# felicityin/zkvm-brainfuck

Hardware: AMD Instinct MI355X
Metric: core-proof wall-time (ms) + NTT HBM GB/s, fibonacci trace 2^22 rows (lower is better)
Workload: dtype u32 (KoalaBear mod-p); 1 GPU; fibo_x4 stdin[255]: 3,767,729 cycles, Cpu trace 2^22 rows, full core proof (84 FRI queries, 16 PoW bits); cycles=3767729, parallelism=replicas x1

## Files before the change

zkvm-brainfuck_amd/csrc/merkle.hip:

```cpp
#include <algorithm>

#include "merkle.h"
#include "poseidon2.h"


namespace bfz {

using namespace kb;

constexpr int MAXSEG = 16;
struct ColList {
  const uint32_t* base[MAXSEG];
  size_t stride[MAXSEG];
  int start[MAXSEG + 1];
  int nseg;
  int n;
  __device__ __forceinline__ const uint32_t* col(int c) const {
    int s = 0;
    while (s + 1 < nseg && c >= start[s + 1]) s++;
    return base[s] + (size_t)(c - start[s]) * stride[s];
  }
};

__device__ __forceinline__ void sponge_cols(uint32_t st[16], const ColList& cl, size_t row) {
  for (int c0 = 0; c0 < cl.n; c0 += 8) {
#pragma unroll
    for (int k = 0; k < 8; k++)
      if (c0 + k < cl.n) st[k] = cl.col(c0 + k)[row];
    poseidon2_permute(st);
  }
}

__global__ __launch_bounds__(256) void k_hash_leaves(ColList cl, size_t r0, size_t count,
                                                     uint32_t* __restrict__ out) {
  const size_t i = (size_t)blockIdx.x * blockDim.x + threadIdx.x;
  if (i >= count) return;
  const size_t r = r0 + i;
  uint32_t st[16];
#pragma unroll
  for (int i = 0; i < 16; i++) st[i] = 0;
  sponge_cols(st, cl, r);
  uint4* o = reinterpret_cast<uint4*>(out + 8 * r);
  o[0] = make_uint4(st[0], st[1], st[2], st[3]);
  o[1] = make_uint4(st[4], st[5], st[6], st[7]);
}

__device__ __forceinline__ void merkle_node(uint32_t st[16], const ColList& cl, int c0, int c1,
                                            size_t j) {
  const int nchunks = (c1 - c0 + 7) >> 3;
  const int nsteps = nchunks ? nchunks + 2 : 1;
  uint32_t d[8];
  for (int step = 0; step < nsteps; step++) {
    if (step == 1) {
#pragma unroll
      for (int i = 0; i < 8; i++) d[i] = st[i];
#pragma unroll
      for (int i = 0; i < 16; i++) st[i] = 0;
    }
    if (step >= 1 && step <= nchunks) {
      const int cb = c0 + 8 * (step - 1);
#pragma unroll
      for (int k = 0; k < 8; k++)
        if (cb + k < c1) st[k] = cl.col(cb + k)[j];
    }
    if (nchunks && step == nchunks + 1) {
#pragma unroll
      for (int i = 0; i < 8; i++) {
        st[8 + i] = st[i];
        st[i] = d[i];
      }
    }
    poseidon2_permute(st);
  }
}

__device__ __forceinline__ void load16(uint32_t st[16], const uint32_t* p) {
  const uint4* in = reinterpret_cast<const uint4*>(p);
  const uint4 a = in[0], b = in[1], c = in[2], d = in[3];
  st[0] = a.x; st[1] = a.y; st[2] = a.z; st[3] = a.w;
  st[4] = b.x; st[5] = b.y; st[6] = b.z; st[7] = b.w;
  st[8] = c.x; st[9] = c.y; st[10] = c.z; st[11] = c.w;
  st[12] = d.x; st[13] = d.y; st[14] = d.z; st[15] = d.w;
}

__device__ __forceinline__ void store8(uint32_t* p, const uint32_t st[16]) {
  uint4* o = reinterpret_cast<uint4*>(p);
  o[0] = make_uint4(st[0], st[1], st[2], st[3]);
  o[1] = make_uint4(st[4], st[5], st[6], st[7]);
}

__global__ __launch_bounds__(256) void k_compress(const uint32_t* __restrict__ prev, size_t j0,
                                                  size_t count, uint32_t* __restrict__ out,
                                                  ColList inj) {
  const size_t i = (size_t)blockIdx.x * blockDim.x + threadIdx.x;
  if (i >= count) return;
  const size_t j = j0 + i;
  uint32_t st[16];
  load16(st, prev + 16 * j);
  merkle_node(st, inj, 0, inj.n, j);
  store8(out + 8 * j, st);
}

__device__ __forceinline__ uint32_t merkle_node_lane(uint32_t v, const ColList& cl, int c0, int c1,
                                                     size_t j, int lane, const LaneConsts& kc) {
  v = poseidon2_permute_lane(v, lane, kc);
  const int nchunks = (c1 - c0 + 7) >> 3;
  if (nchunks) {
    const uint32_t d = v;
    uint32_t h = 0;
    for (int k = 0; k < nchunks; k++) {
      const int col = c0 + 8 * k + lane;
      if (lane < 8 && col < c1) h = cl.col(col)[j];
      h = poseidon2_permute_lane(h, lane, kc);
    }
    const uint32_t hs = dpp<DPP_ROR8>(h);
    v = poseidon2_permute_lane(lane < 8 ? d : hs, lane, kc);
  }
  return v;
}

constexpr int TOP_NODES = 64;
constexpr int TOP_LAYERS = 7;
constexpr size_t LANE_LAYER_MAX = (size_t)1 << 14;
constexpr int MAXTOP = TOP_LAYERS;
struct TopLayers {
  uint32_t* out[MAXTOP];
  int c0[MAXTOP], c1[MAXTOP];
  int n;
};

__global__ __launch_bounds__(1024) void k_compress_top(const uint32_t* __restrict__ prev,
                                                       size_t nlen, ColList inj, TopLayers tl,
                                                       RootChallenge rc, size_t base) {
  __shared__ uint32_t buf[2][TOP_NODES * 8];
  const size_t per = nlen < (size_t)TOP_NODES ? nlen : (size_t)TOP_NODES;
  const size_t g0 = base + (size_t)blockIdx.x * per;
  const int lane = threadIdx.x & 15;
  const LaneConsts kc = lane_consts(lane);
  for (int l = 0; l < tl.n; l++) {
    const size_t m = per >> l, g = g0 >> l;
    const uint32_t* src = buf[(l - 1) & 1];
    uint32_t* dst = buf[l & 1];
    for (size_t j = threadIdx.x >> 4; j < m; j += blockDim.x >> 4) {
      const uint32_t x = l == 0 ? ld_global(prev, 16 * (g + j) + lane) : src[16 * j + lane];
      const uint32_t v = merkle_node_lane(x, inj, tl.c0[l], tl.c1[l], g + j, lane, kc);
      if (lane < 8) {
        tl.out[l][8 * (g + j) + lane] = v;
        dst[8 * j + lane] = v;
      }
    }
    __syncthreads();
  }
  if (rc.state && threadIdx.x < 64) {
    const uint32_t* root = buf[(tl.n - 1) & 1];
    uint32_t v = lane < 8 ? root[lane] : ld_global(rc.state, lane);
    v = poseidon2_permute_lane(v, lane, kc);
    if (threadIdx.x < 16) {
      rc.state[lane] = v;
      if (lane >= 4 && lane < 8) rc.beta->c[7 - lane] = v;
    }
  }
}

__global__ __launch_bounds__(256) void k_compress_lanes(const uint32_t* __restrict__ prev,
                                                        size_t j0, size_t count,
                                                        uint32_t* __restrict__ out, ColList inj) {
  const size_t i = ((size_t)blockIdx.x * blockDim.x + threadIdx.x) >> 4;
  const int lane = threadIdx.x & 15;
  if (i >= count) return;
  const size_t j = j0 + i;
  const uint32_t v = merkle_node_lane(prev[16 * j + lane], inj, 0, inj.n, j, lane, lane_consts(lane));
  if (lane < 8) out[8 * j + lane] = v;
}

__global__ __launch_bounds__(256) void k_hash_rows8_lanes(const uint32_t* __restrict__ rows,
                                                          size_t r0, size_t count,
                                                          uint32_t* __restrict__ out) {
  const size_t i = r0 + (((size_t)blockIdx.x * blockDim.x + threadIdx.x) >> 4);
  const int lane = threadIdx.x & 15;
  if (i >= r0 + count) return;
  const uint32_t v = poseidon2_permute_lane(lane < 8 ? rows[8 * i + lane] : 0u, lane);
  if (lane < 8) out[8 * i + lane] = v;
}

__global__ __launch_bounds__(256) void k_permute_lanes(uint32_t* __restrict__ s, size_t n) {
  const size_t i = ((size_t)blockIdx.x * blockDim.x + threadIdx.x) >> 4;
  const int lane = threadIdx.x & 15;
  if (i >= n) return;
  s[16 * i + lane] = poseidon2_permute_lane(s[16 * i + lane], lane);
}

__global__ __launch_bounds__(256) void k_permute_batch(uint32_t* __restrict__ s, size_t n) {
  const size_t i = (size_t)blockIdx.x * blockDim.x + threadIdx.x;
  if (i >= n) return;
  uint32_t st[16];
#pragma unroll
  for (int k = 0; k < 16; k++) st[k] = s[16 * i + k];
  poseidon2_permute(st);
#pragma unroll
  for (int k = 0; k < 16; k++) s[16 * i + k] = st[k];
}

__global__ __launch_bounds__(256) void k_hash_rows8(const uint32_t* __restrict__ rows, size_t r0,
                                                    size_t count, uint32_t* __restrict__ out) {
  const size_t i = r0 + (size_t)blockIdx.x * blockDim.x + threadIdx.x;
  if (i >= r0 + count) return;
  uint32_t st[16];
  const uint4* in = reinterpret_cast<const uint4*>(rows + 8 * i);
  uint4 a = in[0], b = in[1];
  st[0] = a.x; st[1] = a.y; st[2] = a.z; st[3] = a.w;
  st[4] = b.x; st[5] = b.y; st[6] = b.z; st[7] = b.w;
#pragma unroll
  for (int k = 8; k < 16; k++) st[k] = 0;
  poseidon2_permute(st);
  uint4* o = reinterpret_cast<uint4*>(out + 8 * i);
  o[0] = make_uint4(st[0], st[1], st[2], st[3]);
  o[1] = make_uint4(st[4], st[5], st[6], st[7]);
}

static ColList make_cols(const std::vector<const MatRef*>& ms) {
  ColList cl{};
  cl.n = 0;
  cl.nseg = 0;
  for (const MatRef* m : ms) {
    if (cl.nseg >= MAXSEG) throw std::runtime_error("merkle: too many matrices at one height");
    cl.base[cl.nseg] = m->base;
    cl.stride[cl.nseg] = m->stride ? m->stride : m->height;
    cl.start[cl.nseg] = cl.n;
    cl.nseg++;
    cl.n += m->width;
  }
  cl.start[cl.nseg] = cl.n;
  return cl;
}

static void launch_layer(MerkleTree& t, int L, size_t j0, size_t count,
                         const std::vector<const MatRef*>& grp, hipStream_t st) {
  const uint32_t* prev = t.layers[L - 1].p;
  if (count <= LANE_LAYER_MAX)
    hipLaunchKernelGGL(k_compress_lanes, dim3(ceil_div(16 * count, 256)), dim3(256), 0, st, prev,
                       j0, count, t.layers[L].p, make_cols(grp));
  else {
    const ColList cl = make_cols(grp);
    KernelProbe& probe = p2_probe();
    hipEvent_t ev0 = probe.on ? probe.begin(st) : nullptr;
    hipLaunchKernelGGL(k_compress, dim3(ceil_div(count, 256)), dim3(256), 0, st, prev, j0, count,
                       t.layers[L].p, cl);
    if (probe.on)
      probe.end(ev0, st, (double)count * (cl.n ? 2 + (cl.n + 7) / 8 : 1), cl.n ? "k_compress+inject" : "k_compress");
  }
  KCHECK();
}

static void build_layers(MerkleTree& t, int L0, size_t len, const std::vector<const MatRef*>& sorted,
                         size_t next, hipStream_t st, bool fetch_root = true,
                         RootChallenge rc = {}) {
  const int nl = (int)t.layers.size() - 1;
  int L = L0;
  for (; L <= nl && (len >> 1) > LANE_LAYER_MAX; L++) {
    const size_t nlen = len >> 1;
    std::vector<const MatRef*> grp;
    while (next < sorted.size() && sorted[next]->height == nlen) grp.push_back(sorted[next++]);
    t.layers[L].reset(8 * nlen);
    launch_layer(t, L, 0, nlen, grp, st);
    len = nlen;
  }
  while (L <= nl) {
    const size_t first = len >> 1;
    const int sub = first > (size_t)TOP_NODES ? TOP_LAYERS : log2i(first) + 1;
    TopLayers tl{};
    tl.n = std::min(sub, nl - L + 1);
    std::vector<const MatRef*> all;
    size_t nlen = first;
    for (int l = 0; l < tl.n; l++, nlen >>= 1) {
      tl.c0[l] = 0;
      for (const MatRef* m : all) tl.c0[l] += m->width;
      while (next < sorted.size() && sorted[next]->height == nlen) all.push_back(sorted[next++]);
      tl.c1[l] = 0;
      for (const MatRef* m : all) tl.c1[l] += m->width;
      t.layers[L + l].reset(8 * nlen);
      tl.out[l] = t.layers[L + l].p;
    }
    const unsigned blocks = first > (size_t)TOP_NODES ? (unsigned)(first / TOP_NODES) : 1u;
    const bool root_launch = L + tl.n > nl;
    hipLaunchKernelGGL(k_compress_top, dim3(blocks), dim3(16 * TOP_NODES), 0, st,
                       (const uint32_t*)t.layers[L - 1].p, first, make_cols(all), tl,
                       root_launch ? rc : RootChallenge{}, (size_t)0);
    KCHECK();
    L += tl.n;
    len = first >> (tl.n - 1);
  }
  if (next != sorted.size()) throw std::runtime_error("merkle: non power-of-two heights");
  if (!fetch_root) return;
  fetch(t.root, t.layers[nl].p, 32, st);
}

ShardCtx*& shard_ctx() {
  static ShardCtx* c = nullptr;
  return c;
}

static bool shard_tree(size_t h0) {
  const ShardCtx* c = shard_ctx();
  return c && c->world > 1 && h0 >= (size_t)c->world * SHARD_MIN_LEAVES;
}

template <class Leaves>
static void build_sharded(MerkleTree& t, size_t h0, const std::vector<const MatRef*>& sorted,
                          size_t next, Leaves leaves, hipStream_t st, bool fetch_root,
                          RootChallenge rc = {}) {
  const ShardCtx& c = *shard_ctx();
  const size_t G = (size_t)c.world, k = (size_t)c.rank;
  const int nl = log2i(h0), lg = log2i(G);
  t.sharded_below = nl - lg;
  t.shard_log = lg;
  leaves(k * (h0 / G), h0 / G);
  size_t len = h0;
  int L = 1;
  for (; L <= nl - lg && (len >> 1) / G > LANE_LAYER_MAX; L++) {
    const size_t nlen = len >> 1;
    std::vector<const MatRef*> grp;
    while (next < sorted.size() && sorted[next]->height == nlen) grp.push_back(sorted[next++]);
    t.layers[L].reset(8 * nlen);
    launch_layer(t, L, k * (nlen / G), nlen / G, grp, st);
    len = nlen;
  }
  while (L <= nl - lg) {
    const size_t first = (len >> 1) / G;
    const int sub = first > (size_t)TOP_NODES ? TOP_LAYERS : log2i(first) + 1;
    TopLayers tl{};
    tl.n = std::min(sub, nl - lg - L + 1);
    std::vector<const MatRef*> all;
    size_t nlen = len >> 1;
    for (int l = 0; l < tl.n; l++, nlen >>= 1) {
      tl.c0[l] = 0;
      for (const MatRef* m : all) tl.c0[l] += m->width;
      while (next < sorted.size() && sorted[next]->height == nlen) all.push_back(sorted[next++]);
      tl.c1[l] = 0;
      for (const MatRef* m : all) tl.c1[l] += m->width;
      t.layers[L + l].reset(8 * nlen);
      tl.out[l] = t.layers[L + l].p;
    }
    const unsigned blocks = first > (size_t)TOP_NODES ? (unsigned)(first / TOP_NODES) : 1u;
    hipLaunchKernelGGL(k_compress_top, dim3(blocks), dim3(16 * TOP_NODES), 0, st,
                       (const uint32_t*)t.layers[L - 1].p, first, make_cols(all), tl,
                       RootChallenge{}, k * first);
    KCHECK();
    L += tl.n;
    len >>= tl.n;
  }
  DBuf<uint32_t>& lay = t.layers[nl - lg];
  DBuf<uint32_t> all(8 * G);
  coll_sync(st);
  c.allgather(lay.p + 8 * k, 32, all.p);
  HIP_CHECK(hipMemcpyAsync(lay.p, all.p, 32 * G, hipMemcpyDeviceToDevice, st));
  build_layers(t, nl - lg + 1, G, sorted, next, st, fetch_root, rc);
}

void merkle_build(const std::vector<MatRef>& mats, MerkleTree& t, hipStream_t st, bool fetch_root) {
  if (mats.empty()) throw std::runtime_error("merkle: no matrices");
  t.mats = mats;
  std::vector<const MatRef*> sorted;
  for (const MatRef& m : mats) sorted.push_back(&m);
  std::stable_sort(sorted.begin(), sorted.end(),
                   [](const MatRef* a, const MatRef* b) { return a->height > b->height; });
  const size_t h0 = sorted[0]->height;
  t.layers.clear();
  t.layers.resize(log2i(h0) + 1);
  t.sharded_below = 0;
  size_t next = 0;
  std::vector<const MatRef*> grp;
  while (next < sorted.size() && sorted[next]->height == h0) grp.push_back(sorted[next++]);
  t.layers[0].reset(8 * h0);
  const ColList cl = make_cols(grp);
  auto leaves = [&](size_t r0, size_t count) {
    KernelProbe& probe = p2_probe();
    hipEvent_t ev0 = probe.on ? probe.begin(st) : nullptr;
    hipLaunchKernelGGL(k_hash_leaves, dim3(ceil_div(count, 256)), dim3(256), 0, st, cl, r0,
                       count, t.layers[0].p);
    KCHECK();
    if (probe.on) probe.end(ev0, st, (double)count * ((cl.n + 7) / 8), "k_hash_leaves");
  };
  if (shard_tree(h0)) {
    build_sharded(t, h0, sorted, next, leaves, st, fetch_root);
    return;
  }
  leaves(0, h0);
  build_layers(t, 1, h0, sorted, next, st, fetch_root);
}

static void hash_rows8_range(const uint32_t* rows, size_t r0, size_t count, uint32_t* digests,
                             hipStream_t st) {
  if (count <= LANE_LAYER_MAX)
    hipLaunchKernelGGL(k_hash_rows8_lanes, dim3(ceil_div(16 * count, 256)), dim3(256), 0, st, rows,
                       r0, count, digests);
  else {
    KernelProbe& probe = p2_probe();
    hipEvent_t ev0 = probe.on ? probe.begin(st) : nullptr;
    hipLaunchKernelGGL(k_hash_rows8, dim3(ceil_div(count, 256)), dim3(256), 0, st, rows, r0, count,
                       digests);
    if (probe.on) probe.end(ev0, st, (double)count, "k_hash_rows8");
  }
  KCHECK();
}

void merkle_from_rows8(MerkleTree& t, const uint32_t* rows, size_t h, hipStream_t st,
                       bool fetch_root, RootChallenge rc, bool allow_shard,
                       const std::function<void(size_t, size_t, uint32_t*)>& fused) {
  t.mats = {MatRef{rows, h, 8}};
  t.layers.clear();
  t.layers.resize(log2i(h) + 1);
  t.layers[0].reset(8 * h);
  t.sharded_below = 0;
  auto leaves = [&](size_t r0, size_t count) {
    if (fused) fused(r0, count, t.layers[0].p);
    else hash_rows8_range(rows, r0, count, t.layers[0].p, st);
  };
  if (h < 2) throw std::runtime_error("merkle: rows8 tree needs two leaves");
  if (allow_shard && shard_tree(h)) {
    build_sharded(t, h, {}, 0, leaves, st, fetch_root, rc);
    return;
  }
  leaves(0, h);
  build_layers(t, 1, h, {}, 0, st, fetch_root, rc);
}

void poseidon2_batch(uint32_t* states, size_t n, hipStream_t st) {
  hipLaunchKernelGGL(k_permute_batch, dim3(ceil_div(n, 256)), dim3(256), 0, st, states, n);
  KCHECK();
}

void poseidon2_batch_small(uint32_t* states, size_t n, hipStream_t st) {
  hipLaunchKernelGGL(k_permute_lanes, dim3(ceil_div(16 * n, 256)), dim3(256), 0, st, states, n);
  KCHECK();
}

static PreloadKernels preload_merkle{
    (const void*)&k_hash_leaves,
    (const void*)&k_compress,
    (const void*)&k_compress_top,
    (const void*)&k_compress_lanes,
    (const void*)&k_hash_rows8_lanes,
    (const void*)&k_hash_rows8};

}
```

zkvm-brainfuck_amd/csrc/poseidon2.h:

```cpp
#pragma once
#include "kb.h"

namespace kb {

struct P2Tables {
  uint32_t ext_init[4][16];
  uint32_t ext_term[4][16];
  uint32_t ext_init_r2[4][16];
  uint32_t ext_term_r2[4][16];
  uint32_t internal[13];
  uint32_t diag[16];
  uint32_t dabs[16];
};

constexpr uint32_t RC_RAW[30 * 16] = {
#include "rc_16_30.inc"
};

constexpr uint32_t cinv(uint32_t a) { return cpow(a, P - 2); }
constexpr uint32_t cneg(uint32_t a) { return a ? P - a : 0; }

constexpr P2Tables make_p2_tables() {
  P2Tables t{};
  for (int r = 0; r < 4; r++)
    for (int i = 0; i < 16; i++) {
      t.ext_init[r][i] = to_mont_c(RC_RAW[r * 16 + i] % P);
      t.ext_term[r][i] = to_mont_c(RC_RAW[(17 + r) * 16 + i] % P);
      t.ext_init_r2[r][i] = to_mont_c(t.ext_init[r][i]);
      t.ext_term_r2[r][i] = to_mont_c(t.ext_term[r][i]);
    }
  for (int r = 0; r < 13; r++) t.internal[r] = to_mont_c(RC_RAW[(4 + r) * 16] % P);
  uint32_t d[16] = {cneg(2),        1,          2,         cinv(2),          3,
                    4,              cneg(cinv(2)), cneg(3), cneg(4),          cinv(256),
                    cinv(8),        cinv(1u << 24), cneg(cinv(256)), cneg(cinv(8)), cneg(cinv(16)),
                    cneg(cinv(1u << 24))};
  uint32_t da[16] = {2, 1, 2, cinv(2), 3, 4, cinv(2), 3, 4, cinv(256), cinv(8), cinv(1u << 24),
                     cinv(256), cinv(8), cinv(16), cinv(1u << 24)};
  for (int i = 0; i < 16; i++) {
    t.diag[i] = to_mont_c(d[i]);
    t.dabs[i] = to_mont_c(da[i]);
  }
  return t;
}

constexpr P2Tables P2 = make_p2_tables();

KB_HD uint32_t cube(uint32_t x) {
  const uint64_t t = (uint64_t)x * x;
  const uint32_t m = (uint32_t)t * MU;
  const int32_t x2 = (int32_t)(opaque((uint32_t)(t >> 32)) - (uint32_t)(((uint64_t)m * P) >> 32));
  const int64_t u = (int64_t)x2 * (int64_t)(int32_t)x;
  const uint32_t m2 = (uint32_t)u * MU;
  const int32_t mh = (int32_t)(((int64_t)(int32_t)m2 * (int64_t)P) >> 32);
  const uint32_t r = (uint32_t)((int32_t)(u >> 32) - mh);
  return umin(r, r + P);
}

constexpr uint32_t C32 = (1u << 25) - 2;
KB_HD void mds_light64(uint64_t s[16]) {
#pragma unroll
  for (int b = 0; b < 16; b += 4) {
    const uint64_t x0 = s[b], x1 = s[b + 1], x2 = s[b + 2], x3 = s[b + 3];
    const uint64_t t01 = x0 + x1, t23 = x2 + x3, t0123 = t01 + t23;
    const uint64_t t01123 = t0123 + x1, t01233 = t0123 + x3;
    s[b + 3] = t01233 + (x0 + x0);
    s[b + 1] = t01123 + (x2 + x2);
    s[b + 0] = t01123 + t01;
    s[b + 2] = t01233 + t23;
  }
  uint64_t sums[4];
#pragma unroll
  for (int k = 0; k < 4; k++) sums[k] = (s[k] + s[4 + k]) + (s[8 + k] + s[12 + k]);
#pragma unroll
  for (int i = 0; i < 16; i++) s[i] += sums[i & 3];
}
constexpr int32_t centred(uint32_t x) { return x > P / 2 ? (int32_t)(x - P) : (int32_t)x; }
struct P2Signed {
  int32_t rc_init[4][16];
  int32_t rc_term[4][16];
  int32_t rc_int[13];
  int32_t d[16];
  int32_t k;
};
constexpr P2Signed make_p2_signed() {
  P2Signed t{};
  for (int r = 0; r < 4; r++)
    for (int i = 0; i < 16; i++) {
      t.rc_init[r][i] = centred(P2.ext_init_r2[r][i]);
      t.rc_term[r][i] = centred(P2.ext_term_r2[r][i]);
    }
  for (int r = 0; r < 13; r++) t.rc_int[r] = centred(to_mont_c(P2.internal[r]));
  for (int i = 0; i < 16; i++) t.d[i] = centred(P2.diag[i]);
  t.k = centred(R2);
  return t;
}
constexpr P2Signed P2S = make_p2_signed();

struct P2Pre {
  int32_t init0[16];
  int32_t init[4][16];
  int32_t term[4][16];
};
constexpr uint32_t cmul_mod(uint32_t a, uint32_t b) { return (uint32_t)((uint64_t)a * b % P); }
constexpr void m4_inverse(uint32_t inv[4][4]) {
  constexpr uint32_t m4[4][4] = {{2, 3, 1, 1}, {1, 2, 3, 1}, {1, 1, 2, 3}, {3, 1, 1, 2}};
  uint32_t a[4][8] = {};
  for (int i = 0; i < 4; i++)
    for (int j = 0; j < 4; j++) {
      a[i][j] = m4[i][j];
      a[i][4 + j] = i == j;
    }
  for (int c = 0; c < 4; c++) {
    int piv = c;
    while (a[piv][c] == 0) piv++;
    for (int j = 0; j < 8; j++) {
      const uint32_t t = a[c][j];
      a[c][j] = a[piv][j];
      a[piv][j] = t;
    }
    const uint32_t iv = cpow(a[c][c], P - 2);
    for (int j = 0; j < 8; j++) a[c][j] = cmul_mod(a[c][j], iv);
    for (int i = 0; i < 4; i++)
      if (i != c && a[i][c]) {
        const uint32_t f = a[i][c];
        for (int j = 0; j < 8; j++) a[i][j] = (a[i][j] + P - cmul_mod(f, a[c][j])) % P;
      }
  }
  for (int i = 0; i < 4; i++)
    for (int j = 0; j < 4; j++) inv[i][j] = a[i][4 + j];
}
constexpr void mds_light_inverse(const uint32_t v[16], int32_t out[16]) {
  uint32_t inv[4][4] = {};
  m4_inverse(inv);
  const uint32_t inv5 = cpow(5, P - 2);
  uint32_t w[16] = {};
  for (int k = 0; k < 4; k++) {
    uint64_t sum = 0;
    for (int b = 0; b < 4; b++) sum += v[4 * b + k];
    const uint32_t s5 = cmul_mod((uint32_t)(sum % P), inv5);
    for (int b = 0; b < 4; b++) w[4 * b + k] = (v[4 * b + k] + P - s5) % P;
  }
  for (int b = 0; b < 4; b++)
    for (int i = 0; i < 4; i++) {
      uint64_t acc = 0;
      for (int j = 0; j < 4; j++) acc += (uint64_t)inv[i][j] * w[4 * b + j] % P;
      out[4 * b + i] = centred((uint32_t)(acc % P));
    }
}
constexpr P2Pre make_p2_pre() {
  P2Pre t{};
  mds_light_inverse(P2.ext_init_r2[0], t.init0);
  for (int r = 0; r < 3; r++) {
    mds_light_inverse(P2.ext_init_r2[r + 1], t.init[r]);
    mds_light_inverse(P2.ext_term_r2[r + 1], t.term[r]);
  }
  uint32_t e0[16] = {};
  e0[0] = to_mont_c(P2.internal[0]);
  mds_light_inverse(e0, t.init[3]);
  return t;
}
constexpr P2Pre P2PRE = make_p2_pre();

struct P2Mul {
  int32_t d[16];
  int32_t k;
  int32_t one[16];
  int32_t dd[16];
};
constexpr P2Mul make_p2_mul() {
  P2Mul m{};
  for (int i = 0; i < 16; i++) {
    m.d[i] = P2S.d[i];
    m.one[i] = 1;
    m.dd[i] = centred(to_mont_c(P2.diag[i]));
  }
  m.k = P2S.k;
  return m;
}
#ifdef __HIP_DEVICE_COMPILE__
__constant__ P2Mul P2M_DEV = make_p2_mul();
#define P2M P2M_DEV
#else
constexpr P2Mul P2M_HOST = make_p2_mul();
#define P2M P2M_HOST
#endif
KB_HD int64_t opaque64(int64_t x) {
#ifdef __HIP_DEVICE_COMPILE__
  asm("" : "+v"(x));
#endif
  return x;
}
KB_HD int32_t mred_s(int64_t y) {
  const int32_t m = (int32_t)((uint32_t)y * MU_NEG);
#ifdef __HIP_DEVICE_COMPILE__
  int64_t r;
  uint64_t carry;
  asm("v_mad_i64_i32 %0, %1, %2, %3, %4" : "=v"(r), "=s"(carry) : "v"(m), "s"(P), "v"(y));
  return (int32_t)(r >> 32);
#else
  const uint32_t mh = (uint32_t)(((int64_t)(int32_t)(0u - (uint32_t)m) * (int64_t)P) >> 32);
  return (int32_t)((uint32_t)((uint64_t)y >> 32) - mh);
#endif
}
template <int SH>
KB_HD int64_t lshl_add64(int64_t a, int64_t b) {
#ifdef __HIP_DEVICE_COMPILE__
  int64_t r;
  asm("v_lshl_add_u64 %0, %1, %2, %3" : "=v"(r) : "v"(a), "n"(SH), "v"(b));
  return r;
#else
  return (int64_t)(((uint64_t)a << SH) + (uint64_t)b);
#endif
}
KB_HD int64_t cube_s(int32_t a) {
  const int64_t A = (int64_t)a * a;
  return (int64_t)mred_s(A) * a;
}
KB_HD int64_t fold_s(int64_t u) {
  return (int64_t)(int32_t)(u >> 32) * (int64_t)C32 + (int64_t)(uint32_t)u;
}
KB_HD void external_rounds_pre(const int32_t a[16], int64_t y[16], const int32_t (&K)[4][16]) {
  uint64_t* u = reinterpret_cast<uint64_t*>(y);
#pragma unroll
  for (int r = 0; r < 4; r++) {
#pragma unroll
    for (int i = 0; i < 16; i++) {
      const int32_t x = r ? mred_s(y[i]) : a[i];
      const int64_t c3 = (int64_t)mred_s((int64_t)x * x) * x + K[r][i];
      y[i] = fold_s(c3);
    }
    mds_light64(u);
  }
}
KB_HD void poseidon2_permute(uint32_t s[16]) {
  int64_t y[16];
  int32_t t[16];
#pragma unroll
  for (int i = 0; i < 16; i++) y[i] = (int64_t)((uint64_t)s[i] * C32) + P2PRE.init0[i];
  mds_light64(reinterpret_cast<uint64_t*>(y));
#pragma unroll
  for (int i = 0; i < 16; i++) t[i] = mred_s(y[i]);
  external_rounds_pre(t, y, P2PRE.init);
#pragma unroll
  for (int i = 0; i < 16; i++) t[i] = mred_s(y[i]);
  int64_t u1 = t[1], u2 = t[2], u4 = t[4], u5 = t[5];
#pragma unroll
  for (int r = 0; r < 13; r++) {
    const int32_t c = mred_s(cube_s(t[0]));
    int64_t part[2];
    part[0] = (int64_t)P2M.one[0] * c;
    part[0] = (int64_t)P2M.one[3] * t[3] + part[0];
    part[0] = (int64_t)P2M.one[6] * t[6] + part[0];
    part[0] = (int64_t)P2M.one[7] * t[7] + part[0];
    part[0] = part[0] + u1;
    part[0] = part[0] + u2;
    part[1] = (int64_t)P2M.one[8] * t[8];
#pragma unroll
    for (int i = 9; i < 16; i++) part[1] = (int64_t)P2M.one[i] * t[i] + part[1];
    part[1] = part[1] + u4;
    part[1] = part[1] + u5;
    const int32_t sp = mred_s(part[0] + part[1]);
    const int64_t q = opaque64((int64_t)P2M.k * sp);
    if (r < 12) {
      const int64_t tr = (int64_t)mred_s(q);
      t[0] = mred_s((int64_t)P2M.d[0] * c + (q + P2S.rc_int[r + 1]));
#pragma unroll
      for (int i = 3; i < 16; i++)
        if (i != 4 && i != 5) t[i] = mred_s((int64_t)P2M.d[i] * t[i] + q);
      u1 = lshl_add64<0>(u1, tr);
      u2 = lshl_add64<1>(u2, tr);
      u4 = lshl_add64<0>(lshl_add64<1>(u4, u4), tr);
      u5 = lshl_add64<2>(u5, tr);
    } else {
      t[0] = mred_s((int64_t)P2M.d[0] * c + (q + P2S.rc_term[0][0]));
#pragma unroll
      for (int i = 3; i < 16; i++)
        if (i != 4 && i != 5) t[i] = mred_s((int64_t)P2M.d[i] * t[i] + (q + P2S.rc_term[0][i]));
      t[1] = mred_s((int64_t)P2M.dd[1] * mred_s(u1) + (q + P2S.rc_term[0][1]));
      t[2] = mred_s((int64_t)P2M.dd[2] * mred_s(u2) + (q + P2S.rc_term[0][2]));
      t[4] = mred_s((int64_t)P2M.dd[4] * mred_s(u4) + (q + P2S.rc_term[0][4]));
      t[5] = mred_s((int64_t)P2M.dd[5] * mred_s(u5) + (q + P2S.rc_term[0][5]));
    }
  }
  external_rounds_pre(t, y, P2PRE.term);
#pragma unroll
  for (int i = 0; i < 16; i++) {
    const uint32_t r = (uint32_t)mred_s(y[i]);
    s[i] = umin(r, r + P);
  }
}
template <int CTRL>
__device__ __forceinline__ uint32_t dpp(uint32_t v) {
  return (uint32_t)__builtin_amdgcn_update_dpp(0, (int)v, CTRL, 0xf, 0xf, false);
}
constexpr int DPP_QROT1 = 0x39, DPP_QROT2 = 0x4E, DPP_QROT3 = 0x93;
constexpr int DPP_ROR1 = 0x121, DPP_ROR2 = 0x122, DPP_ROR4 = 0x124, DPP_ROR8 = 0x128;

template <int CTRL>
__device__ __forceinline__ int64_t dpp64(int64_t v) {
  const uint32_t lo = (uint32_t)__builtin_amdgcn_mov_dpp((int)(uint32_t)(uint64_t)v, CTRL, 0xf, 0xf, false);
  const uint32_t hi = (uint32_t)__builtin_amdgcn_mov_dpp((int)(uint32_t)((uint64_t)v >> 32), CTRL, 0xf, 0xf, false);
  return (int64_t)(((uint64_t)hi << 32) | lo);
}
__device__ __forceinline__ int64_t mds_light64_lane(int64_t y) {
  const int64_t a1 = dpp64<DPP_QROT1>(y), a2 = dpp64<DPP_QROT2>(y), a3 = dpp64<DPP_QROT3>(y);
  const int64_t p1 = lshl_add64<1>(y, a1);
  const int64_t m = lshl_add64<0>(p1, lshl_add64<0>(lshl_add64<1>(a1, a2), a3));
  const int64_t t = lshl_add64<0>(m, dpp64<DPP_ROR8>(m));
  return lshl_add64<0>(m, lshl_add64<0>(t, dpp64<DPP_ROR4>(t)));
}
__device__ __forceinline__ int64_t sum_lanes16_64(int64_t v) {
  v = lshl_add64<0>(v, dpp64<DPP_ROR1>(v));
  v = lshl_add64<0>(v, dpp64<DPP_ROR2>(v));
  v = lshl_add64<0>(v, dpp64<DPP_ROR4>(v));
  return lshl_add64<0>(v, dpp64<DPP_ROR8>(v));
}

struct LaneConsts {
  int32_t kin[4], kte[3];
  int32_t init0, d, rct;
};
__device__ __forceinline__ LaneConsts lane_consts(int lane) {
  LaneConsts k;
#pragma unroll
  for (int r = 0; r < 4; r++) k.kin[r] = P2PRE.init[r][lane];
#pragma unroll
  for (int r = 0; r < 3; r++) k.kte[r] = P2PRE.term[r][lane];
  k.init0 = P2PRE.init0[lane];
  k.d = P2M.d[lane];
  k.rct = P2S.rc_term[0][lane];
  return k;
}

__device__ __forceinline__ int64_t external_rounds_lane(int32_t x, const int32_t* K, int nk) {
  int64_t y = 0;
#pragma unroll
  for (int r = 0; r < 4; r++) {
    if (r) x = mred_s(y);
    const int64_t c3 = (int64_t)mred_s((int64_t)x * x) * x + (r < nk ? K[r] : 0);
    y = mds_light64_lane(fold_s(c3));
  }
  return y;
}
__device__ __forceinline__ uint32_t poseidon2_permute_lane(uint32_t v, int lane,
                                                           const LaneConsts& kc) {
  int64_t y = mds_light64_lane((int64_t)((uint64_t)v * C32) + kc.init0);
  y = external_rounds_lane(mred_s(y), kc.kin, 4);
  int32_t t = mred_s(y);
#pragma unroll
  for (int r = 0; r < 13; r++) {
    const int32_t c = mred_s(cube_s(t));
    const int32_t u = lane == 0 ? c : t;
    const int32_t sp = mred_s(sum_lanes16_64((int64_t)u));
    const int64_t q = opaque64((int64_t)P2S.k * sp);
    const int32_t add = r < 12 ? (lane == 0 ? P2S.rc_int[r + 1] : 0) : kc.rct;
    t = mred_s((int64_t)kc.d * u + (q + add));
  }
  y = external_rounds_lane(t, kc.kte, 3);
  const uint32_t r = (uint32_t)mred_s(y);
  return umin(r, r + P);
}
__device__ __forceinline__ uint32_t poseidon2_permute_lane(uint32_t v, int lane) {
  return poseidon2_permute_lane(v, lane, lane_consts(lane));
}

}
```

Measured before the change: 25.78 ms.

## Stream Merkle column pointers and skip unused Poseidon2 prologue/epilogue lanes

Replaces the per-column segment search with a walking pointer over column segments, and uses 32-bit byte offsets for loads. Adds a Poseidon2 variant that skips the capacity multiplies when the capacity is known zero, and skips the final reduction of state words that will be overwritten by the next absorb. This cuts integer work in the leaf-hashing and compress kernels. The 32-bit offset needs a new height limit of 2^30 rows, and unread state words are left as undefined registers.

```diff
diff --git a/zkvm-brainfuck_amd/csrc/merkle.hip b/zkvm-brainfuck_amd/csrc/merkle.hip
--- a/zkvm-brainfuck_amd/csrc/merkle.hip
+++ b/zkvm-brainfuck_amd/csrc/merkle.hip
@@ -9,25 +9,92 @@
 using namespace kb;
 
 constexpr int MAXSEG = 16;
+struct ColSeg {
+  const uint32_t* base;
+  size_t stride;
+  int n;
+};
 struct ColList {
-  const uint32_t* base[MAXSEG];
-  size_t stride[MAXSEG];
-  int start[MAXSEG + 1];
+  ColSeg seg[MAXSEG];
   int nseg;
   int n;
-  __device__ __forceinline__ const uint32_t* col(int c) const {
-    int s = 0;
-    while (s + 1 < nseg && c >= start[s + 1]) s++;
-    return base[s] + (size_t)(c - start[s]) * stride[s];
-  }
 };
 
-__device__ __forceinline__ void sponge_cols(uint32_t st[16], const ColList& cl, size_t row) {
-  for (int c0 = 0; c0 < cl.n; c0 += 8) {
-#pragma unroll
-    for (int k = 0; k < 8; k++)
-      if (c0 + k < cl.n) st[k] = cl.col(c0 + k)[row];
-    poseidon2_permute(st);
+struct ColWalk {
+  const uint32_t* p;
+  size_t stride;
+  int left;
+  int s;
+  __device__ __forceinline__ void enter(const ColList& cl, int seg) {
+    s = seg;
+    p = nullptr;
+    stride = 0;
+    left = 0;
+    if (seg < cl.nseg) {
+      p = cl.seg[seg].base;
+      stride = cl.seg[seg].stride;
+      left = cl.seg[seg].n;
+    }
+  }
+  __device__ __forceinline__ const uint32_t* next(const ColList& cl) {
+    const uint32_t* r = p;
+    if (left > 1) {
+      left--;
+      p += stride;
+    } else if (s + 1 < cl.nseg) {
+      enter(cl, s + 1);
+    }
+    return r;
+  }
+  __device__ __forceinline__ const uint32_t* next_lanes(const ColList& cl, int m, int lane) {
+    const uint32_t* r = nullptr;
+    for (int k0 = 0; k0 < m && left > 0;) {
+      const int take = m - k0 < left ? m - k0 : left;
+      const int k = lane - k0;
+      if (k >= 0 && k < take) r = p + (size_t)k * stride;
+      k0 += take;
+      if (left > take) {
+        left -= take;
+        p += (size_t)take * stride;
+      } else {
+        enter(cl, s + 1);
+      }
+    }
+    return r;
+  }
+};
+
+__device__ __forceinline__ uint32_t ld_col(const uint32_t* col, uint32_t off4) {
+  return *reinterpret_cast<const uint32_t*>(reinterpret_cast<const char*>(col) + off4);
+}
+
+__device__ __forceinline__ void load_chunk(uint32_t nx[8], ColWalk& w, const ColList& cl,
+                                           uint32_t off4) {
+#pragma unroll
+  for (int k = 0; k < 8; k++) nx[k] = ld_col(w.next(cl), off4);
+}
+
+__device__ __forceinline__ void take_chunk(uint32_t st[16], const uint32_t nx[8], int m) {
+  if (m == 8) {
+#pragma unroll
+    for (int k = 0; k < 8; k++) st[k] = nx[k];
+  } else {
+#pragma unroll
+    for (int k = 0; k < 7; k++) st[k] = k < m ? nx[k] : st[k];
+  }
+}
+
+__device__ __forceinline__ void sponge_cols(uint32_t st[16], const ColList& cl, uint32_t off4) {
+  ColWalk w;
+  w.enter(cl, 0);
+  bool first = true;
+  for (int rest = cl.n; rest > 0; first = false) {
+    const int m = rest < 8 ? rest : 8;
+    uint32_t nx[8];
+    load_chunk(nx, w, cl, off4);
+    take_chunk(st, nx, m);
+    rest -= m;
+    poseidon2_permute_ends(st, first, rest < 8, rest > 0);
   }
 }
 
@@ -39,18 +106,21 @@
   uint32_t st[16];
 #pragma unroll
   for (int i = 0; i < 16; i++) st[i] = 0;
-  sponge_cols(st, cl, r);
+  sponge_cols(st, cl, (uint32_t)r * 4u);
   uint4* o = reinterpret_cast<uint4*>(out + 8 * r);
   o[0] = make_uint4(st[0], st[1], st[2], st[3]);
   o[1] = make_uint4(st[4], st[5], st[6], st[7]);
 }
 
-__device__ __forceinline__ void merkle_node(uint32_t st[16], const ColList& cl, int c0, int c1,
-                                            size_t j) {
-  const int nchunks = (c1 - c0 + 7) >> 3;
+__device__ __forceinline__ void merkle_node(uint32_t st[16], const ColList& cl, uint32_t off4) {
+  const int nchunks = (cl.n + 7) >> 3;
   const int nsteps = nchunks ? nchunks + 2 : 1;
+  ColWalk w;
+  w.enter(cl, 0);
   uint32_t d[8];
+  int rest = cl.n;
   for (int step = 0; step < nsteps; step++) {
+    bool lo = true, hi = false;
     if (step == 1) {
 #pragma unroll
       for (int i = 0; i < 8; i++) d[i] = st[i];
@@ -58,10 +128,15 @@
       for (int i = 0; i < 16; i++) st[i] = 0;
     }
     if (step >= 1 && step <= nchunks) {
-      const int cb = c0 + 8 * (step - 1);
-#pragma unroll
-      for (int k = 0; k < 8; k++)
-        if (cb + k < c1) st[k] = cl.col(cb + k)[j];
+      const int m = rest < 8 ? rest : 8;
+      uint32_t nx[8];
+      load_chunk(nx, w, cl, off4);
+      take_chunk(st, nx, m);
+      rest -= m;
+      if (rest > 0) {
+        lo = rest < 8;
+        hi = true;
+      }
     }
     if (nchunks && step == nchunks + 1) {
 #pragma unroll
@@ -70,7 +145,7 @@
         st[i] = d[i];
       }
     }
-    poseidon2_permute(st);
+    poseidon2_permute_ends(st, step == 1, lo, hi);
   }
 }
 
@@ -97,20 +172,22 @@
   const size_t j = j0 + i;
   uint32_t st[16];
   load16(st, prev + 16 * j);
-  merkle_node(st, inj, 0, inj.n, j);
+  merkle_node(st, inj, (uint32_t)j * 4u);
   store8(out + 8 * j, st);
 }
 
-__device__ __forceinline__ uint32_t merkle_node_lane(uint32_t v, const ColList& cl, int c0, int c1,
+__device__ __forceinline__ uint32_t merkle_node_lane(uint32_t v, const ColList& cl, int s0, int nc,
                                                      size_t j, int lane, const LaneConsts& kc) {
+  ColWalk w;
+  w.enter(cl, s0);
   v = poseidon2_permute_lane(v, lane, kc);
-  const int nchunks = (c1 - c0 + 7) >> 3;
-  if (nchunks) {
+  if (nc > 0) {
     const uint32_t d = v;
     uint32_t h = 0;
-    for (int k = 0; k < nchunks; k++) {
-      const int col = c0 + 8 * k + lane;
-      if (lane < 8 && col < c1) h = cl.col(col)[j];
+    for (int rest = nc; rest > 0; rest -= 8) {
+      const int m = rest < 8 ? rest : 8;
+      const uint32_t* col = w.next_lanes(cl, m, lane);
+      if (lane < m && col) h = col[j];
       h = poseidon2_permute_lane(h, lane, kc);
     }
     const uint32_t hs = dpp<DPP_ROR8>(h);
@@ -125,7 +202,7 @@
 constexpr int MAXTOP = TOP_LAYERS;
 struct TopLayers {
   uint32_t* out[MAXTOP];
-  int c0[MAXTOP], c1[MAXTOP];
+  int s0[MAXTOP], nc[MAXTOP];
   int n;
 };
 
@@ -143,7 +220,7 @@
     uint32_t* dst = buf[l & 1];
     for (size_t j = threadIdx.x >> 4; j < m; j += blockDim.x >> 4) {
       const uint32_t x = l == 0 ? ld_global(prev, 16 * (g + j) + lane) : src[16 * j + lane];
-      const uint32_t v = merkle_node_lane(x, inj, tl.c0[l], tl.c1[l], g + j, lane, kc);
+      const uint32_t v = merkle_node_lane(x, inj, tl.s0[l], tl.nc[l], g + j, lane, kc);
       if (lane < 8) {
         tl.out[l][8 * (g + j) + lane] = v;
         dst[8 * j + lane] = v;
@@ -223,15 +300,26 @@
   cl.n = 0;
   cl.nseg = 0;
   for (const MatRef* m : ms) {
+    if (m->width <= 0) continue;
     if (cl.nseg >= MAXSEG) throw std::runtime_error("merkle: too many matrices at one height");
-    cl.base[cl.nseg] = m->base;
-    cl.stride[cl.nseg] = m->stride ? m->stride : m->height;
-    cl.start[cl.nseg] = cl.n;
+    if (m->height > ((size_t)1 << 30)) throw std::runtime_error("merkle: matrix taller than 2^30");
+    cl.seg[cl.nseg].base = m->base;
+    cl.seg[cl.nseg].stride = m->stride ? m->stride : m->height;
+    cl.seg[cl.nseg].n = m->width;
     cl.nseg++;
     cl.n += m->width;
   }
-  cl.start[cl.nseg] = cl.n;
   return cl;
+}
+
+static void top_layer_cols(TopLayers& tl, int l, std::vector<const MatRef*>& all,
+                           const std::vector<const MatRef*>& sorted, size_t& next, size_t nlen) {
+  tl.s0[l] = make_cols(all).nseg;
+  tl.nc[l] = 0;
+  while (next < sorted.size() && sorted[next]->height == nlen) {
+    tl.nc[l] += sorted[next]->width;
+    all.push_back(sorted[next++]);
+  }
 }
 
 static void launch_layer(MerkleTree& t, int L, size_t j0, size_t count,
@@ -273,11 +361,7 @@
     std::vector<const MatRef*> all;
     size_t nlen = first;
     for (int l = 0; l < tl.n; l++, nlen >>= 1) {
-      tl.c0[l] = 0;
-      for (const MatRef* m : all) tl.c0[l] += m->width;
-      while (next < sorted.size() && sorted[next]->height == nlen) all.push_back(sorted[next++]);
-      tl.c1[l] = 0;
-      for (const MatRef* m : all) tl.c1[l] += m->width;
+      top_layer_cols(tl, l, all, sorted, next, nlen);
       t.layers[L + l].reset(8 * nlen);
       tl.out[l] = t.layers[L + l].p;
     }
@@ -333,11 +417,7 @@
     std::vector<const MatRef*> all;
     size_t nlen = len >> 1;
     for (int l = 0; l < tl.n; l++, nlen >>= 1) {
-      tl.c0[l] = 0;
-      for (const MatRef* m : all) tl.c0[l] += m->width;
-      while (next < sorted.size() && sorted[next]->height == nlen) all.push_back(sorted[next++]);
-      tl.c1[l] = 0;
-      for (const MatRef* m : all) tl.c1[l] += m->width;
+      top_layer_cols(tl, l, all, sorted, next, nlen);
       t.layers[L + l].reset(8 * nlen);
       tl.out[l] = t.layers[L + l].p;
     }
diff --git a/zkvm-brainfuck_amd/csrc/poseidon2.h b/zkvm-brainfuck_amd/csrc/poseidon2.h
--- a/zkvm-brainfuck_amd/csrc/poseidon2.h
+++ b/zkvm-brainfuck_amd/csrc/poseidon2.h
@@ -57,7 +57,7 @@
 }
 
 constexpr uint32_t C32 = (1u << 25) - 2;
-KB_HD void mds_light64(uint64_t s[16]) {
+KB_HD void mds_light64_blocks(uint64_t s[16], uint64_t sums[4]) {
 #pragma unroll
   for (int b = 0; b < 16; b += 4) {
     const uint64_t x0 = s[b], x1 = s[b + 1], x2 = s[b + 2], x3 = s[b + 3];
@@ -68,9 +68,12 @@
     s[b + 0] = t01123 + t01;
     s[b + 2] = t01233 + t23;
   }
+#pragma unroll
+  for (int k = 0; k < 4; k++) sums[k] = (s[k] + s[4 + k]) + (s[8 + k] + s[12 + k]);
+}
+KB_HD void mds_light64(uint64_t s[16]) {
   uint64_t sums[4];
-#pragma unroll
-  for (int k = 0; k < 4; k++) sums[k] = (s[k] + s[4 + k]) + (s[8 + k] + s[12 + k]);
+  mds_light64_blocks(s, sums);
 #pragma unroll
   for (int i = 0; i < 16; i++) s[i] += sums[i & 3];
 }
@@ -219,7 +222,8 @@
 KB_HD int64_t fold_s(int64_t u) {
   return (int64_t)(int32_t)(u >> 32) * (int64_t)C32 + (int64_t)(uint32_t)u;
 }
-KB_HD void external_rounds_pre(const int32_t a[16], int64_t y[16], const int32_t (&K)[4][16]) {
+KB_HD void external_rounds_pre(const int32_t a[16], int64_t y[16], const int32_t (&K)[4][16],
+                               uint64_t* sums = nullptr) {
   uint64_t* u = reinterpret_cast<uint64_t*>(y);
 #pragma unroll
   for (int r = 0; r < 4; r++) {
@@ -229,17 +233,37 @@
       const int64_t c3 = (int64_t)mred_s((int64_t)x * x) * x + K[r][i];
       y[i] = fold_s(c3);
     }
-    mds_light64(u);
-  }
-}
-KB_HD void poseidon2_permute(uint32_t s[16]) {
+    if (r == 3 && sums) mds_light64_blocks(u, sums);
+    else mds_light64(u);
+  }
+}
+KB_HD void p2_prologue(const uint32_t s[16], int32_t t[16]) {
   int64_t y[16];
-  int32_t t[16];
 #pragma unroll
   for (int i = 0; i < 16; i++) y[i] = (int64_t)((uint64_t)s[i] * C32) + P2PRE.init0[i];
   mds_light64(reinterpret_cast<uint64_t*>(y));
 #pragma unroll
   for (int i = 0; i < 16; i++) t[i] = mred_s(y[i]);
+}
+KB_HD void p2_prologue_cap0(const uint32_t s[16], int32_t t[16]) {
+  int64_t y[16];
+#pragma unroll
+  for (int i = 0; i < 8; i++) y[i] = (int64_t)((uint64_t)s[i] * C32) + P2PRE.init0[i];
+#pragma unroll
+  for (int i = 8; i < 16; i++) y[i] = P2PRE.init0[i];
+  mds_light64(reinterpret_cast<uint64_t*>(y));
+#pragma unroll
+  for (int i = 0; i < 16; i++) t[i] = mred_s(y[i]);
+}
+template <int I0, int I1>
+KB_HD void p2_epilogue(uint32_t s[16], const int64_t y[16], const uint64_t sums[4]) {
+#pragma unroll
+  for (int i = I0; i < I1; i++) {
+    const uint32_t r = (uint32_t)mred_s((int64_t)((uint64_t)y[i] + sums[i & 3]));
+    s[i] = umin(r, r + P);
+  }
+}
+KB_HD void p2_core(int32_t t[16], int64_t y[16], uint64_t sums[4]) {
   external_rounds_pre(t, y, P2PRE.init);
 #pragma unroll
   for (int i = 0; i < 16; i++) t[i] = mred_s(y[i]);
@@ -282,11 +306,41 @@
       t[5] = mred_s((int64_t)P2M.dd[5] * mred_s(u5) + (q + P2S.rc_term[0][5]));
     }
   }
-  external_rounds_pre(t, y, P2PRE.term);
-#pragma unroll
-  for (int i = 0; i < 16; i++) {
-    const uint32_t r = (uint32_t)mred_s(y[i]);
-    s[i] = umin(r, r + P);
+  external_rounds_pre(t, y, P2PRE.term, sums);
+}
+KB_HD void poseidon2_permute(uint32_t s[16]) {
+  int64_t y[16];
+  uint64_t sums[4];
+  int32_t t[16];
+  p2_prologue(s, t);
+  p2_core(t, y, sums);
+  p2_epilogue<0, 16>(s, y, sums);
+}
+KB_HD uint32_t unread_word() {
+  uint32_t x = 0;
+#ifdef __HIP_DEVICE_COMPILE__
+  asm volatile("" : "=v"(x));
+#endif
+  return x;
+}
+KB_HD void poseidon2_permute_ends(uint32_t s[16], bool cap0, bool lo, bool hi) {
+  int64_t y[16];
+  uint64_t sums[4];
+  int32_t t[16];
+  if (cap0) p2_prologue_cap0(s, t);
+  else p2_prologue(s, t);
+  p2_core(t, y, sums);
+  if (lo) {
+    p2_epilogue<0, 8>(s, y, sums);
+  } else {
+#pragma unroll
+    for (int i = 0; i < 8; i++) s[i] = unread_word();
+  }
+  if (hi) {
+    p2_epilogue<8, 16>(s, y, sums);
+  } else {
+#pragma unroll
+    for (int i = 8; i < 16; i++) s[i] = unread_word();
   }
 }
 template <int CTRL>
```

Measured after the change: 25.51 ms (median of 6 runs). 1.0% less time.
